# RaptorMai/online-continual-learning

Hardware: NVIDIA H100
Metric: replay-step images/sec (ASER+SCR, ResNet18, CIFAR100) (higher is better)
Workload: dtype f32

## Files before the change

### online-continual-learning_b200/csrc/conv_tc.cu

```cuda
#include <stdlib.h>

#include "conv.cuh"
#include "umma.cuh"

namespace b200ocl {
namespace {

constexpr int TC_THREADS = 128;
constexpr int A_TILE = 128 * 32;

__device__ __forceinline__ void cp_async16(void* smem_dst, const void* gmem_src) {
  const unsigned int s = static_cast<unsigned int>(__cvta_generic_to_shared(smem_dst));
  asm volatile("cp.async.cg.shared.global [%0], [%1], 16;\n" ::"r"(s), "l"(gmem_src));
}

template <int R>
__device__ __forceinline__ void promote(float (&acc)[R], const float (&tmp)[R]) {
#pragma unroll
  for (int i = 0; i < R; ++i) acc[i] += tmp[i];
}

template <int NT>
__device__ __forceinline__ void issue_kblock(float (&d)[2][NT / 2], const float* sAh, const float* sAl, const float* sB) {
  constexpr int B_TILE = NT * 32;
#pragma unroll
  for (int h = 0; h < 2; ++h) {
    const uint64_t dAh = umma::make_smem_desc_sw128(umma::smem_u32(sAh + h * 64 * 32));
    const uint64_t dAl = umma::make_smem_desc_sw128(umma::smem_u32(sAl + h * 64 * 32));
    const uint64_t dBh = umma::make_smem_desc_sw128(umma::smem_u32(sB));
    const uint64_t dBl = umma::make_smem_desc_sw128(umma::smem_u32(sB + B_TILE));
#pragma unroll
    for (int k = 0; k < 4; ++k) {
      const uint64_t adv = (uint64_t)(k * 2);
      umma::mma_tf32_ss<NT>(d[h], dAh + adv, dBh + adv, k > 0 ? 1u : 0u);
      umma::mma_tf32_ss<NT>(d[h], dAh + adv, dBl + adv, 1u);
      umma::mma_tf32_ss<NT>(d[h], dAl + adv, dBh + adv, 1u);
    }
  }
}

template <int NT>
__global__ void __launch_bounds__(TC_THREADS) conv_tc_kernel(ConvArgs a) {
  constexpr int B_TILE = NT * 32;
  constexpr int STAGE_F = 2 * A_TILE + 2 * B_TILE;
  extern __shared__ __align__(1024) unsigned char smem_raw[];
  float* stage0 = reinterpret_cast<float*>(smem_raw);
  __shared__ bool is_last;

  const int tid = threadIdx.x;
  const int bn = a.tc_bn;
  const int n0 = blockIdx.y * bn;
  const int KB = a.tc_kb;
  const int m = blockIdx.x * 128 + tid;
  const bool valid = m < a.M;
  const int hw = a.Hout * a.Wout;
  const int img = valid ? m / hw : 0;
  const int rem = valid ? m - img * hw : 0;
  const int py = rem / a.Wout, px = rem - py * a.Wout;
  const float* wimg = a.w_tc + (size_t)blockIdx.y * KB * 2 * B_TILE;

  float accf[2][NT / 2], tmp[2][NT / 2];
#pragma unroll
  for (int h = 0; h < 2; ++h)
#pragma unroll
    for (int i = 0; i < NT / 2; ++i) accf[h][i] = 0.f;

  int tap = 0, ci = 0;
  const float* tap_src = nullptr;
  auto set_tap = [&]() {
    const int kh = tap / 3, kw = tap - kh * 3;
    const int iy = py + kh - 1, ix = px + kw - 1;
    const bool ok = valid && tap < 9 && (unsigned)iy < (unsigned)a.Hin && (unsigned)ix < (unsigned)a.Win;
    tap_src = ok ? a.in + ((size_t)(img * a.Hin + iy) * a.Win + ix) * a.CK : nullptr;
  };
  set_tap();

  for (int kb = 0; kb < KB; ++kb) {
    const int s = kb & 1;
    float* sAh = stage0 + s * STAGE_F;
    float* sAl = sAh + A_TILE;
    float* sB = sAl + A_TILE;
    const float* bsrc = wimg + (size_t)kb * 2 * B_TILE;
#pragma unroll
    for (int i = 0; i < (2 * B_TILE / 4) / TC_THREADS; ++i)
      cp_async16(sB + (tid + i * TC_THREADS) * 4, bsrc + (tid + i * TC_THREADS) * 4);
// ... 114 lines not shown
      __syncthreads();
      if (is_last) {
        __threadfence();
        const int groups = TC_THREADS / bn;
        const int ch = tid % bn, grp = tid / bn;
        double* s_fin = reinterpret_cast<double*>(stage0);
        __syncthreads();
        if (grp < groups) {
          double s4[4] = {0.0, 0.0, 0.0, 0.0}, q4[4] = {0.0, 0.0, 0.0, 0.0};
          unsigned int b = grp;
          for (; b + 3 * groups < gridDim.x; b += 4 * groups) {
#pragma unroll
            for (int u = 0; u < 4; ++u) {
              const double2 pv = __ldcg(reinterpret_cast<const double2*>(a.stat_part + ((size_t)(b + u * groups) * a.CN + n0 + ch) * 2));
              s4[u] += pv.x;
              q4[u] += pv.y;
            }
          }
          for (; b < gridDim.x; b += groups) {
            const double2 pv = __ldcg(reinterpret_cast<const double2*>(a.stat_part + ((size_t)b * a.CN + n0 + ch) * 2));
            s4[0] += pv.x;
            q4[0] += pv.y;
          }
          s_fin[(grp * bn + ch) * 2 + 0] = (s4[0] + s4[1]) + (s4[2] + s4[3]);
          s_fin[(grp * bn + ch) * 2 + 1] = (q4[0] + q4[1]) + (q4[2] + q4[3]);
        }
        __syncthreads();
        if (tid < bn) {
          double S = 0.0, Q = 0.0;
          for (int g = 0; g < groups; ++g) {
            S += s_fin[(g * bn + tid) * 2 + 0];
            Q += s_fin[(g * bn + tid) * 2 + 1];
          }
          const double cnt = (double)a.M;
          const double mean = S / cnt;
          double var = Q / cnt - mean * mean;
          if (var < 0.0) var = 0.0;
          const int c = n0 + tid;
          a.save_mean[c] = (float)mean;
          a.save_invstd[c] = (float)(1.0 / sqrt(var + (double)a.eps));
          const double unbiased = (a.M > 1) ? var * cnt / (cnt - 1.0) : var;
          a.run_mean[c] = (1.f - a.momentum) * a.run_mean[c] + a.momentum * (float)mean;
          a.run_var[c] = (1.f - a.momentum) * a.run_var[c] + a.momentum * (float)unbiased;
        }
      }
    }
  }
}

template <int NT>
int launch_tc(const ConvArgs& a, cudaStream_t stream) {
  constexpr size_t smem = (size_t)2 * (2 * A_TILE + 2 * NT * 32) * sizeof(float) + 1024;
  static bool configured_dev[B200OCL_MAX_DEVICES] = {};
  bool& configured = configured_dev[b200ocl::device_slot()];
  if (!configured) {
    B200OCL_CUDA(cudaFuncSetAttribute(conv_tc_kernel<NT>, cudaFuncAttributeMaxDynamicSharedMemorySize, (int)smem));
    configured = true;
  }
  dim3 grid((a.M + 127) / 128, a.CN / a.tc_bn);
  B200OCL_PROF(a.flip ? "conv_tc_dgrad" : (a.mode == CONV_EVAL ? "conv_tc_eval" : "conv_tc_train"),
               2.0 * a.M * (double)a.CN * a.CK * 9.0, stream);
  conv_tc_kernel<NT><<<grid, TC_THREADS, smem, stream>>>(a);
  B200OCL_LAUNCHED();
  return B200OCL_OK;
}

}

bool conv_tc_eligible(const ConvArgs& a) {
  static int enabled = -1;
  if (enabled < 0) {
    const char* e = getenv("B200OCL_TC");
    enabled = (e && e[0] == '0') ? 0 : 1;
  }
  if (!enabled || !a.w_tc || a.ks != 3 || a.stride != 1 || a.transposed || a.CK % 20 != 0) return false;
  if (a.Hin != a.Hout || a.Win != a.Wout) return false;
  const long ctas = (long)((a.M + 127) / 128) * (a.CN / a.tc_bn);
  if (ctas < sm_count() / 4) return false;
  if (a.CK == 20 && a.CN == 20 && ctas > 2L * sm_count()) return false;
  return true;
}

int launch_conv_tc(const ConvArgs& a, cudaStream_t stream) {
  const int nt = a.tc_bn <= 20 ? 32 : (a.tc_bn <= 40 ? 48 : 80);
  if (nt == 32) return launch_tc<32>(a, stream);
  if (nt == 48) return launch_tc<48>(a, stream);
  return launch_tc<80>(a, stream);
}

}
```

### online-continual-learning_b200/csrc/conv_tcp.cu

```cuda
#include <stdlib.h>

#include "conv.cuh"
#include "umma.cuh"

namespace b200ocl {
namespace {

constexpr int TP_THREADS = 32 * 13;
constexpr int TP_LOADER_WARP = 9;
constexpr int TP_PS_MAX = 3;
constexpr int TP_BS_MAX = 6;
constexpr int TP_LD_MAX = 13;
constexpr int TP_CONSUMER_WARPS = 8;

using umma::mbar_expect_tx;
using umma::bulk_g2s;

struct TileGeom {
  int wp, pp;
  int tiles_m;
  int prow;
  int pbytes;
};
__host__ __device__ inline TileGeom tile_geom(int N, int H, int W) {
  TileGeom g;
  g.wp = W + 2;
  g.pp = (H + 2) * (W + 2);
  const long last = (long)(N - 1) * g.pp + (long)(H - 1) * g.wp + (W - 1);
  g.tiles_m = (int)(last / 128) + 1;
  g.prow = 128 + 2 * g.wp + 2;
  g.pbytes = (g.prow * 128 + 1023) / 1024 * 1024;
  return g;
}

template <int NT, int KS>
__device__ __forceinline__ void issue_tap(float (&d)[NT / 2], uint64_t dAh, uint64_t dAl, uint64_t dBh, uint64_t dBl) {
  umma::fence();
#pragma unroll
  for (int k = 0; k < KS; ++k) {
    const uint64_t adv = (uint64_t)(k * 2);
    umma::mma_tf32_ss<NT>(d, dAh + adv, dBh + adv, k > 0 ? 1u : 0u);
    umma::mma_tf32_ss<NT>(d, dAh + adv, dBl + adv, 1u);
    umma::mma_tf32_ss<NT>(d, dAl + adv, dBh + adv, 1u);
  }
  umma::commit();
  umma::wait<0>();
  umma::fence_regs(d);
}

template <int NT>
__global__ void __launch_bounds__(TP_THREADS, 1) conv_tcp_kernel(ConvArgs a) {
  constexpr int B_BLOCK = 2 * NT * 32;
  constexpr int R = NT / 2;
  extern __shared__ __align__(1024) unsigned char smem_raw[];
  unsigned char* patch0 = smem_raw;
  __shared__ __align__(8) uint64_t pfull[TP_PS_MAX], pempty[TP_PS_MAX], bfull[9], bempty[TP_BS_MAX];
  __shared__ bool is_last;
  __shared__ int s_fail;
  __shared__ float s_coef[3 * 80];

  const int tid = threadIdx.x, warp = tid >> 5;
  const int bn = a.tp_bn;
  const int n0 = blockIdx.y * bn;
  const int slices = a.tp_slices;
  const TileGeom G = tile_geom(a.N, a.Hin, a.Win);
  const int PS = a.tp_ps, BS = a.tp_bs;
  const int taps_n = a.ks * a.ks;
  const bool one_tap = taps_n == 1;
  float* sB = reinterpret_cast<float*>(smem_raw + (size_t)PS * 2 * G.pbytes);
  const bool resident = (slices == 1 && NT == 32);
  const int b_slots = resident ? 9 : BS;
  float* s_t = sB + (size_t)b_slots * B_BLOCK;
  float* s_acc = s_t + 128 * (bn + 1);

  if (tid == 0) {
    for (int i = 0; i < TP_PS_MAX; ++i) {
      umma::mbar_init(&pfull[i], 128);
      umma::mbar_init(&pempty[i], TP_CONSUMER_WARPS);
    }
    for (int i = 0; i < 9; ++i) umma::mbar_init(&bfull[i], 1);
    for (int i = 0; i < TP_BS_MAX; ++i) umma::mbar_init(&bempty[i], TP_CONSUMER_WARPS);
    umma::fence_mbar_init();
    s_fail = 0;
  }
  __syncthreads();
  const float* wimg = a.w_tp + (size_t)blockIdx.y * slices * taps_n * B_BLOCK;

  if (warp >= TP_LOADER_WARP) {
    const int lt = tid - 32 * TP_LOADER_WARP;
    int pc = 0;
    for (int tile = blockIdx.x; tile < G.tiles_m; tile += gridDim.x) {
      for (int sl = 0; sl < slices; ++sl, ++pc) {
        const int ch_valid = min(32, a.CK - sl * 32);
        const int nch = 2 * ((ch_valid + 7) / 8);
        const int ch = lt & 7, r0 = lt >> 3;
        const int nrow = G.prow;
        const bool ch_live = ch < nch, ch_real = ch * 4 < ch_valid;
        float4 v[TP_LD_MAX];
        int img, yp, xp;
        {
          const int sp = tile * 128 + r0;
          img = sp / G.pp;
          const int rem = sp - img * G.pp;
          yp = rem / G.wp;
          xp = rem - yp * G.wp;
        }
        const int hp = a.Hin + 2;
#pragma unroll
        for (int i = 0; i < TP_LD_MAX; ++i) {
          v[i] = make_float4(0.f, 0.f, 0.f, 0.f);
          const int ri = r0 + 16 * i;
          if (ch_real && ri < nrow) {
            const int y = yp - 1, x = xp - 1;
            if (img < a.N && (unsigned)y < (unsigned)a.Hin && (unsigned)x < (unsigned)a.Win)
              v[i] = __ldg(reinterpret_cast<const float4*>(a.in + ((size_t)(img * a.Hin + y) * a.Win + x) * a.CK + sl * 32) + ch);
          }
          xp += 16;
          while (xp >= G.wp) {
            xp -= G.wp;
            if (++yp == hp) {
              yp = 0;
              ++img;
            }
          }
        }
        const int ps = pc % PS;
        if (!umma::mbar_wait(&pempty[ps], (uint32_t)(((pc / PS) & 1) ^ 1))) s_fail = 1;
        float* ph = reinterpret_cast<float*>(patch0 + (size_t)ps * 2 * G.pbytes);
        float* pl = ph + G.pbytes / 4;
        if (ch_live) {
#pragma unroll
          for (int i = 0; i < TP_LD_MAX; ++i) {
            const int ri = r0 + 16 * i;
            if (ri < nrow) {
              float4 h, l;
              umma::split_tf32(v[i].x, h.x, l.x); umma::split_tf32(v[i].y, h.y, l.y);
              umma::split_tf32(v[i].z, h.z, l.z); umma::split_tf32(v[i].w, h.w, l.w);
              const int off = umma::sw128_offset_f32(ri, ch);
              *reinterpret_cast<float4*>(ph + off) = h;
              *reinterpret_cast<float4*>(pl + off) = l;
            }
          }
        }
        umma::fence_proxy_async_smem();
        umma::mbar_arrive(&pfull[ps]);
      }
    }
  } else if (warp == TP_LOADER_WARP - 1) {
    const uint32_t bytes = (uint32_t)(B_BLOCK * sizeof(float));
    if (resident) {
      if (umma::elect_one_sync()) {
        for (int b = 0; b < taps_n; ++b) {
          mbar_expect_tx(&bfull[b], bytes);
// ... 147 lines not shown
            }
          }
          esync();
          double* s_p = reinterpret_cast<double*>(s_t);
          if (part < parts) {
            s_p[(part * bn + ch) * 2 + 0] = S;
            s_p[(part * bn + ch) * 2 + 1] = Q;
          }
          esync();
          if (et < bn) {
            double Ss = 0.0, Qs = 0.0;
            for (int pp = 0; pp < parts; ++pp) {
              Ss += s_p[(pp * bn + et) * 2 + 0];
              Qs += s_p[(pp * bn + et) * 2 + 1];
            }
            statS += Ss;
            statQ += Qs;
          }
          esync();
        }
      }
    }
    if (epi && a.mode == CONV_TRAIN) {
      if (et < bn) {
        double* dst = a.stat_part + ((size_t)blockIdx.x * a.CN + n0 + et) * 2;
        dst[0] = statS;
        dst[1] = statQ;
      }
      __threadfence();
      esync();
      if (et == 0) is_last = (atomicAdd(a.counter + blockIdx.y, 1u) == gridDim.x - 1);
      esync();
      if (is_last) {
        __threadfence();
        const int groups = 128 / bn;
        const int ch = et % bn, grp = et / bn;
        double* s_fin = reinterpret_cast<double*>(s_t);
        if (grp < groups) {
          double S = 0.0, Q = 0.0;
          unsigned int b = grp;
          for (; b + 3 * groups < gridDim.x; b += 4 * groups) {
            double2 pv[4];
#pragma unroll
            for (int u = 0; u < 4; ++u)
              pv[u] = __ldcg(reinterpret_cast<const double2*>(a.stat_part + ((size_t)(b + u * groups) * a.CN + n0 + ch) * 2));
            S += (pv[0].x + pv[1].x) + (pv[2].x + pv[3].x);
            Q += (pv[0].y + pv[1].y) + (pv[2].y + pv[3].y);
          }
          for (; b < gridDim.x; b += groups) {
            const double2 pv = __ldcg(reinterpret_cast<const double2*>(a.stat_part + ((size_t)b * a.CN + n0 + ch) * 2));
            S += pv.x;
            Q += pv.y;
          }
          s_fin[(grp * bn + ch) * 2 + 0] = S;
          s_fin[(grp * bn + ch) * 2 + 1] = Q;
        }
        esync();
        if (et < bn) {
          double Sm = 0.0, Q = 0.0;
          for (int gq = 0; gq < groups; ++gq) {
            Sm += s_fin[(gq * bn + et) * 2 + 0];
            Q += s_fin[(gq * bn + et) * 2 + 1];
          }
          const double cnt = (double)a.M;
          const double mean = Sm / cnt;
          double var = Q / cnt - mean * mean;
          if (var < 0.0) var = 0.0;
          const int c = n0 + et;
          a.save_mean[c] = (float)mean;
          a.save_invstd[c] = (float)(1.0 / sqrt(var + (double)a.eps));
          const double unbiased = (a.M > 1) ? var * cnt / (cnt - 1.0) : var;
          a.run_mean[c] = (1.f - a.momentum) * a.run_mean[c] + a.momentum * (float)mean;
          a.run_var[c] = (1.f - a.momentum) * a.run_var[c] + a.momentum * (float)unbiased;
        }
      }
    }
  }
  __syncthreads();
  if (s_fail && tid == 0) a.out[(size_t)n0] = __int_as_float(0x7fc00000);
}

template <int NT>
size_t tcp_smem_bytes(const TileGeom& G, int bn, int slices, int ps, int bs) {
  const int b_slots = (slices == 1 && NT == 32) ? 9 : bs;
  return (size_t)ps * 2 * G.pbytes + (size_t)b_slots * 2 * NT * 32 * sizeof(float) +
         (size_t)128 * (bn + 1) * sizeof(float) + (size_t)128 * (NT + 1) * sizeof(float) + 1024;
}

template <int NT>
int launch_tcp(ConvArgs a, cudaStream_t stream) {
  const TileGeom G0 = tile_geom(a.N, a.Hin, a.Win);
  const size_t limit = 227 * 1024 - 4096;
  a.tp_ps = 3; a.tp_bs = 6;
  if (tcp_smem_bytes<NT>(G0, a.tp_bn, a.tp_slices, a.tp_ps, a.tp_bs) > limit) a.tp_bs = 4;
  if (tcp_smem_bytes<NT>(G0, a.tp_bn, a.tp_slices, a.tp_ps, a.tp_bs) > limit) { a.tp_ps = 2; a.tp_bs = 6; }
  const size_t smem = tcp_smem_bytes<NT>(G0, a.tp_bn, a.tp_slices, a.tp_ps, a.tp_bs);
  static size_t configured_dev[B200OCL_MAX_DEVICES] = {};
  size_t& configured = configured_dev[b200ocl::device_slot()];
  if (smem > configured) {
    B200OCL_CUDA(cudaFuncSetAttribute(conv_tcp_kernel<NT>, cudaFuncAttributeMaxDynamicSharedMemorySize, (int)smem));
    configured = smem;
  }
  const TileGeom G = tile_geom(a.N, a.Hin, a.Win);
  const int n_tiles = a.CN / a.tp_bn;
  int gx = sm_count() / n_tiles;
  if (gx < 1) gx = 1;
  if (gx > G.tiles_m) gx = G.tiles_m;
  const int rounds = (G.tiles_m + gx - 1) / gx;
  gx = (G.tiles_m + rounds - 1) / rounds;
  B200OCL_PROF("conv_tcp",
               2.0 * a.M * (double)a.CN * a.CK * 9.0, stream);
  conv_tcp_kernel<NT><<<dim3(gx, n_tiles), TP_THREADS, smem, stream>>>(a);
  B200OCL_LAUNCHED();
  return B200OCL_OK;
}

}

bool conv_tcp_mode_allowed(const ConvArgs& a) {
  static int modes = -1;
  if (modes < 0) {
    const char* m = getenv("B200OCL_TCP_MODES");
    modes = (m && m[0] >= '0' && m[0] <= '7') ? (m[0] - '0') : 5;
  }
  const int bit = a.mode == CONV_EVAL ? 1 : (a.mode == CONV_TRAIN ? 2 : 4);
  return (modes & bit) != 0;
}

bool conv_tcp_eligible(const ConvArgs& a) {
  const char* e = getenv("B200OCL_TCP");
  const char* e2 = getenv("B200OCL_TC");
  const bool enabled = !((e && e[0] == '0') || (e2 && e2[0] == '0'));
  if (!enabled || !a.w_tp || a.transposed || a.CK % 4 != 0) return false;
  if (!((a.ks == 3 && a.pad == 1) || (a.ks == 1 && a.pad == 0))) return false;
  if (a.stride != 1 && (a.stride != 2 || a.flip)) return false;
  if (a.Hout != (a.Hin + 2 * a.pad - a.ks) / a.stride + 1 || a.Wout != (a.Win + 2 * a.pad - a.ks) / a.stride + 1) return false;
  if (128 + 2 * (a.Win + 2) + 2 > 16 * TP_LD_MAX) return false;
  if ((long)a.N * (a.Hin + 2) * (a.Win + 2) > 2000000000L) return false;
  if (a.tp_bn <= 0 || a.tp_bn > 40 || a.CN % a.tp_bn != 0) return false;
  return true;
}

int launch_conv_tcp(const ConvArgs& a, cudaStream_t stream) {
  if (a.tp_bn <= 20) return launch_tcp<32>(a, stream);
  return launch_tcp<48>(a, stream);
}

}
```

### online-continual-learning_b200/csrc/net_plan.cuh

```cuda
#pragma once
#include <stddef.h>
#include <string.h>

#include "../../include/b200ocl.h"

namespace b200ocl {

constexpr int NET_MAX_CONV = 20;
constexpr int NET_MAX_LIN = 3;
constexpr float NET_BN_EPS = 1e-5f;
constexpr float NET_BN_MOMENTUM = 0.1f;

struct ConvL {
  int cin, cout, ks, stride, pad;
  int hin, win, hout, wout;
  size_t w_off;
  size_t pkf_off;
  size_t pkd_off;
  size_t act_off;
  size_t tc_f_off, tc_d_off;
  int tc_kb_f, tc_kb_d;
  int tc_bn_f, tc_bn_d;
  size_t tp_f_off, tp_d_off;
  int tp_sl_f, tp_sl_d;
  int tp_bn_f, tp_bn_d;
};

inline int tc_nt(int bn) { return bn <= 20 ? 32 : (bn <= 40 ? 48 : 80); }
struct BnL {
  int c;
  size_t g_off, b_off;
  size_t stat_off;
  size_t save_off;
};
struct LinL {
  int in, out;
  size_t w_off, b_off;
};
struct BlockL {
  int c1, c2, sc;
};

struct NetPlan {
  int n_conv;
  ConvL conv[NET_MAX_CONV];
  BnL bn[NET_MAX_CONV];
  BlockL blk[8];
  int n_lin;
  LinL lin[NET_MAX_LIN];
  int head;
  int in_h, in_w;
  int final_h, final_w;
  int pooled_h, pooled_w;
  int dim_in;
  int out_dim;
  size_t n_params, n_packed, n_stats, n_bn_channels;
  size_t act_per_image;
  size_t max_act_per_image;
};

inline int conv_out(int x, int ks, int stride, int pad) { return (x + 2 * pad - ks) / stride + 1; }

inline void conv_pack_layout(ConvL& c, size_t& pk, bool tp_all = false) {
  const int cin = c.cin, cout = c.cout, ks = c.ks, stride = c.stride, hin = c.hin, win = c.win;
  c.pkf_off = pk; pk += (size_t)cout * cin * ks * ks;
  c.pkd_off = pk; pk += (size_t)cout * cin * ks * ks;
  c.tc_kb_f = c.tc_kb_d = c.tp_sl_f = c.tp_sl_d = 0;
  if (ks == 3 && stride == 1 && cin % 20 == 0) {
    c.tc_bn_f = cout < 80 ? cout : 80;
    c.tc_bn_d = cin < 80 ? cin : 80;
    c.tc_kb_f = (9 * cin + 31) / 32;
    c.tc_kb_d = (9 * cout + 31) / 32;
    c.tc_f_off = pk; pk += (size_t)(cout / c.tc_bn_f) * c.tc_kb_f * 2 * tc_nt(c.tc_bn_f) * 32;
    c.tc_d_off = pk; pk += (size_t)(cin / c.tc_bn_d) * c.tc_kb_d * 2 * tc_nt(c.tc_bn_d) * 32;
  }
  if (cin % 20 == 0 && win <= 37 && ((ks == 3 && c.pad == 1) || (ks == 1 && c.pad == 0)) &&
      (tp_all || (ks == 3 && stride == 1))) {
    const int taps = ks * ks;
    c.tp_bn_f = cout < 40 ? cout : 40;
    c.tp_sl_f = (cin + 31) / 32;
    c.tp_f_off = pk; pk += (size_t)(cout / c.tp_bn_f) * c.tp_sl_f * taps * 2 * tc_nt(c.tp_bn_f) * 32;
    if (ks == 3 && stride == 1) {
      c.tp_bn_d = cin < 40 ? cin : 40;
      c.tp_sl_d = (cout + 31) / 32;
      c.tp_d_off = pk; pk += (size_t)(cin / c.tp_bn_d) * c.tp_sl_d * 9 * 2 * tc_nt(c.tp_bn_d) * 32;
    }
  }
}

inline int build_plan(const b200ocl_net_desc& d, NetPlan& p) {
  memset(&p, 0, sizeof(p));
  if (d.nf != 20 || d.in_h < 8 || d.in_w < 8 || d.head < 0 || d.head > 3) return B200OCL_EUNSUPPORTED;
  p.head = d.head;
  p.in_h = d.in_h;
  p.in_w = d.in_w;
  size_t off = 0, pk = 0, st = 0, sv = 0, act = 0, max_act = 0;
  int nc = 0;
  auto add_conv = [&](int cin, int cout, int ks, int stride, int hin, int win) {
    ConvL& c = p.conv[nc];
    c.cin = cin; c.cout = cout; c.ks = ks; c.stride = stride; c.pad = (ks == 3) ? 1 : 0;
    c.hin = hin; c.win = win;
    c.hout = conv_out(hin, ks, stride, c.pad);
    c.wout = conv_out(win, ks, stride, c.pad);
    c.w_off = off; off += (size_t)cout * cin * ks * ks;
    conv_pack_layout(c, pk);
    c.act_off = act;
    const size_t a = (size_t)c.hout * c.wout * cout;
    act += a;
    if (a > max_act) max_act = a;
    BnL& b = p.bn[nc];
    b.c = cout;
// ... 60 lines not shown
```

### online-continual-learning_b200/csrc/tc_selftest.cu

```cuda
#include "common.cuh"
#include "umma.cuh"

namespace b200ocl {
namespace {

__global__ void __launch_bounds__(128) wgmma_selftest_kernel(const float* __restrict__ A, const float* __restrict__ B,
                                                             float* __restrict__ D, int N, int K, int mode) {
  extern __shared__ __align__(1024) unsigned char smem_raw[];
  float* sAh = reinterpret_cast<float*>(smem_raw);
  float* sAl = sAh + 64 * 32;
  float* sBh = sAl + 64 * 32;
  float* sBl = sBh + 16 * 32;
  const int tid = threadIdx.x;
  for (int h = 0; h < 2; ++h)
    for (int q = 0; q < N / 16; ++q) {
      float d[8];
#pragma unroll
      for (int i = 0; i < 8; ++i) d[i] = 0.f;
      for (int kb = 0; kb < K / 32; ++kb) {
        for (int idx = tid; idx < (64 + 16) * 8; idx += 128) {
          const int r = idx >> 3, c = idx & 7;
          const bool is_a = r < 64;
          const float* src = is_a ? A + (size_t)(64 * h + r) * K : B + (size_t)(16 * q + r - 64) * K;
          const float4 v = *reinterpret_cast<const float4*>(src + kb * 32 + c * 4);
          float4 hi, lo;
          umma::split_tf32(v.x, hi.x, lo.x); umma::split_tf32(v.y, hi.y, lo.y);
          umma::split_tf32(v.z, hi.z, lo.z); umma::split_tf32(v.w, hi.w, lo.w);
          const int off = umma::sw128_offset_f32(is_a ? r : r - 64, c);
          *reinterpret_cast<float4*>((is_a ? sAh : sBh) + off) = (mode == 0) ? v : hi;
          *reinterpret_cast<float4*>((is_a ? sAl : sBl) + off) = lo;
        }
        umma::fence_proxy_async_smem();
        __syncthreads();
        const uint64_t dAh = umma::make_smem_desc_sw128(umma::smem_u32(sAh));
        const uint64_t dAl = umma::make_smem_desc_sw128(umma::smem_u32(sAl));
        const uint64_t dBh = umma::make_smem_desc_sw128(umma::smem_u32(sBh));
        const uint64_t dBl = umma::make_smem_desc_sw128(umma::smem_u32(sBl));
        umma::fence_regs(d);
        umma::fence();
#pragma unroll
        for (int k = 0; k < 4; ++k) {
          const uint64_t adv = (uint64_t)(k * 2);
          umma::mma_tf32_ss<16>(d, dAh + adv, dBh + adv, (kb > 0 || k > 0) ? 1u : 0u);
          if (mode == 1) {
            umma::mma_tf32_ss<16>(d, dAh + adv, dBl + adv, 1u);
            umma::mma_tf32_ss<16>(d, dAl + adv, dBh + adv, 1u);
          }
        }
        umma::commit();
        umma::wait<0>();
        umma::fence_regs(d);
        __syncthreads();
      }
#pragma unroll
      for (int i = 0; i < 8; ++i)
        D[(size_t)(64 * h + umma::frag_row(tid, i)) * N + 16 * q + umma::frag_col(tid, i)] = d[i];
    }
}

__global__ void __launch_bounds__(128) wgmma_window_kernel(const float* __restrict__ P, const float* __restrict__ B,
                                                           float* __restrict__ D, int rows, int start_row, int sbo_rows,
                                                           int base_off_mode, int N) {
  extern __shared__ __align__(1024) unsigned char smem_raw[];
  float* sP = reinterpret_cast<float*>(smem_raw);
  float* sB = sP + (size_t)((rows + 7) / 8 * 8) * 32;
  const int tid = threadIdx.x;
  for (int idx = tid; idx < rows * 8; idx += 128) {
    const int r = idx >> 3, c = idx & 7;
    *reinterpret_cast<float4*>(sP + umma::sw128_offset_f32(r, c)) = *reinterpret_cast<const float4*>(P + (size_t)r * 32 + c * 4);
  }
  for (int idx = tid; idx < N * 8; idx += 128) {
    const int r = idx >> 3, c = idx & 7;
    *reinterpret_cast<float4*>(sB + umma::sw128_offset_f32(r, c)) = *reinterpret_cast<const float4*>(B + (size_t)r * 32 + c * 4);
  }
  umma::fence_proxy_async_smem();
  __syncthreads();
  for (int h = 0; h < 2; ++h) {
    const int row0 = start_row + 8 * h * sbo_rows;
    uint64_t dA = umma::make_smem_desc_sw128(umma::smem_u32(sP) + (uint32_t)row0 * 128u);
    dA &= ~((uint64_t)0x3FFF << 32);
    dA |= (uint64_t)(((uint32_t)sbo_rows * 128u >> 4) & 0x3FFF) << 32;
    if (base_off_mode == 1) dA |= (uint64_t)(row0 & 7) << 49;
    for (int q = 0; q < N / 16; ++q) {
      const uint64_t dB = umma::make_smem_desc_sw128(umma::smem_u32(sB + q * 16 * 32));
      float d[8];
      umma::fence();
#pragma unroll
      for (int k = 0; k < 4; ++k) {
        const uint64_t adv = (uint64_t)(k * 2);
        umma::mma_tf32_ss<16>(d, dA + adv, dB + adv, k > 0 ? 1u : 0u);
      }
      umma::commit();
      umma::wait<0>();
      umma::fence_regs(d);
#pragma unroll
      for (int i = 0; i < 8; ++i)
        D[(size_t)(64 * h + umma::frag_row(tid, i)) * N + 16 * q + umma::frag_col(tid, i)] = d[i];
    }
  }
}

}
}

extern "C" int b200ocl_selftest_umma_tf32(const float* A, const float* B, float* D, int N, int K, int mode, int* status,
                                          void* stream_) {
  using namespace b200ocl;
  cudaStream_t stream = static_cast<cudaStream_t>(stream_);
  B200OCL_CHECK_ARG(A && B && D && status, "null pointer");
  B200OCL_CHECK_ARG(N >= 16 && N <= 256 && N % 16 == 0 && K >= 32 && K % 32 == 0, "need N in [16,256] %16, K %32");
  const size_t smem = (size_t)(2 * 64 * 32 + 2 * 16 * 32) * sizeof(float) + 1024;
  B200OCL_CUDA(cudaMemsetAsync(status, 0, sizeof(int), stream));
  wgmma_selftest_kernel<<<1, 128, smem, stream>>>(A, B, D, N, K, mode);
  B200OCL_LAUNCHED();
  return B200OCL_OK;
}

extern "C" int b200ocl_selftest_umma_window(const float* P, const float* B, float* D, int rows, int start_row,
                                            int sbo_rows, int base_off_mode, int N, int* status, void* stream_) {
  using namespace b200ocl;
  cudaStream_t stream = static_cast<cudaStream_t>(stream_);
  B200OCL_CHECK_ARG(P && B && D && status, "null pointer");
  B200OCL_CHECK_ARG(N >= 16 && N <= 256 && N % 16 == 0, "need N in [16,256] %16");
  B200OCL_CHECK_ARG(rows > 0 && rows <= 1024 && start_row >= 0 && sbo_rows > 0 &&
                        start_row + 15 * sbo_rows + 8 <= rows,
                    "window exceeds the patch");
  const size_t smem = (size_t)((rows + 7) / 8 * 8 + 256) * 32 * sizeof(float) + 1024;
  B200OCL_CUDA(cudaFuncSetAttribute(wgmma_window_kernel, cudaFuncAttributeMaxDynamicSharedMemorySize, (int)smem));
  B200OCL_CUDA(cudaMemsetAsync(status, 0, sizeof(int), stream));
  wgmma_window_kernel<<<1, 128, smem, stream>>>(P, B, D, rows, start_row, sbo_rows, base_off_mode, N);
  B200OCL_LAUNCHED();
  return B200OCL_OK;
}
```

### online-continual-learning_b200/csrc/umma.cuh

```cuda
#pragma once
#include <stdint.h>

namespace b200ocl {
namespace umma {

__device__ __forceinline__ uint32_t smem_u32(const void* p) {
  return static_cast<uint32_t>(__cvta_generic_to_shared(p));
}

__device__ __forceinline__ int sw128_offset_f32(int row, int chunk16) {
  return (row >> 3) * 256 + (row & 7) * 32 + ((chunk16 ^ (row & 7)) << 2);
}

__device__ __forceinline__ int frag_row(int t, int i) { return ((t >> 5) << 4) + ((t & 31) >> 2) + ((i & 2) << 2); }
__device__ __forceinline__ int frag_col(int t, int i) { return ((i >> 2) << 3) + ((t & 3) << 1) + (i & 1); }

__device__ __forceinline__ uint64_t make_smem_desc_sw128(uint32_t smem_addr) {
  uint64_t d = 0;
  d |= (uint64_t)((smem_addr >> 4) & 0x3FFF);
  d |= (uint64_t)1 << 16;
  d |= (uint64_t)((1024 >> 4) & 0x3FFF) << 32;
  d |= (uint64_t)1 << 62;
  return d;
}

__device__ __forceinline__ void fence() { asm volatile("wgmma.fence.sync.aligned;\n" ::: "memory"); }
__device__ __forceinline__ void commit() { asm volatile("wgmma.commit_group.sync.aligned;\n" ::: "memory"); }
template <int N>
__device__ __forceinline__ void wait() { asm volatile("wgmma.wait_group.sync.aligned %0;\n" ::"n"(N) : "memory"); }
template <int R>
__device__ __forceinline__ void fence_regs(float (&d)[R]) {
#pragma unroll
  for (int i = 0; i < R; ++i) asm volatile("" : "+f"(d[i])::"memory");
}
__device__ __forceinline__ void fence_proxy_async_smem() { asm volatile("fence.proxy.async.shared::cta;\n" ::); }

__device__ __forceinline__ void mbar_init(uint64_t* bar, uint32_t count) {
  asm volatile("mbarrier.init.shared::cta.b64 [%0], %1;\n" ::"r"(smem_u32(bar)), "r"(count));
}
__device__ __forceinline__ void fence_mbar_init() { asm volatile("fence.mbarrier_init.release.cluster;\n" ::); }
__device__ __forceinline__ bool mbar_wait(uint64_t* bar, uint32_t parity, uint32_t max_spins = (1u << 24)) {
  const uint32_t addr = smem_u32(bar);
#pragma unroll 1
  for (uint32_t i = 0; i < max_spins; ++i) {
    uint32_t done;
    asm volatile(
        "{\n\t.reg .pred p;\n\t"
        "mbarrier.try_wait.parity.shared::cta.b64 p, [%1], %2;\n\t"
        "selp.u32 %0, 1, 0, p;\n\t}\n"
        : "=r"(done)
        : "r"(addr), "r"(parity)
        : "memory");
    if (done) return true;
  }
  return false;
}
__device__ __forceinline__ void mbar_arrive(uint64_t* bar) {
  asm volatile("mbarrier.arrive.shared::cta.b64 _, [%0];\n" ::"r"(smem_u32(bar)) : "memory");
}

__device__ __forceinline__ void mbar_expect_tx(uint64_t* bar, uint32_t bytes) {
  asm volatile("mbarrier.arrive.expect_tx.shared::cta.b64 _, [%0], %1;\n" ::"r"(smem_u32(bar)), "r"(bytes)
               : "memory");
}
__device__ __forceinline__ void bulk_g2s(void* smem_dst, const void* gmem_src, uint32_t bytes, uint64_t* bar) {
  asm volatile(
      "cp.async.bulk.shared::cluster.global.mbarrier::complete_tx::bytes [%0], [%1], %2, [%3];\n" ::"r"(
          smem_u32(smem_dst)),
      "l"(gmem_src), "r"(bytes), "r"(smem_u32(bar))
      : "memory");
}

__device__ __forceinline__ bool elect_one_sync() {
  uint32_t pred;
  asm volatile(
      "{\n\t.reg .pred P;\n\t"
      "elect.sync _|P, 0xffffffff;\n\t"
      "selp.u32 %0, 1, 0, P;\n\t}\n"
      : "=r"(pred));
  return pred != 0;
}

template <int N>
__device__ __forceinline__ void mma_tf32_ss(float (&d)[N / 2], uint64_t desc_a, uint64_t desc_b, uint32_t accumulate);
template <int N>
__device__ __forceinline__ void mma_tf32_rs(float (&d)[N / 2], const uint32_t (&a)[4], uint64_t desc_b, uint32_t accumulate);

template <>
__device__ __forceinline__ void mma_tf32_ss<16>(float (&d)[8], uint64_t desc_a, uint64_t desc_b, uint32_t accumulate) {
  asm volatile(
      "{\n\t.reg .pred p;\n\t"
      "setp.ne.b32 p, %10, 0;\n\t"
      "wgmma.mma_async.sync.aligned.m64n16k8.f32.tf32.tf32 {%0,%1,%2,%3,%4,%5,%6,%7}, %8, %9, p, 1, 1;\n\t}\n"
      : "+f"(d[0]), "+f"(d[1]), "+f"(d[2]), "+f"(d[3]), "+f"(d[4]), "+f"(d[5]), "+f"(d[6]), "+f"(d[7])
      : "l"(desc_a), "l"(desc_b), "r"(accumulate));
}

template <>
__device__ __forceinline__ void mma_tf32_ss<32>(float (&d)[16], uint64_t desc_a, uint64_t desc_b, uint32_t accumulate) {
  asm volatile(
      "{\n\t.reg .pred p;\n\t"
      "setp.ne.b32 p, %18, 0;\n\t"
      "wgmma.mma_async.sync.aligned.m64n32k8.f32.tf32.tf32 {%0,%1,%2,%3,%4,%5,%6,%7,%8,%9,%10,%11,%12,%13,%14,%15}, %16, %17, p, 1, 1;\n\t}\n"
      : "+f"(d[0]), "+f"(d[1]), "+f"(d[2]), "+f"(d[3]), "+f"(d[4]), "+f"(d[5]), "+f"(d[6]), "+f"(d[7]), "+f"(d[8]), "+f"(d[9]), "+f"(d[10]), "+f"(d[11]), "+f"(d[12]), "+f"(d[13]), "+f"(d[14]), "+f"(d[15])
      : "l"(desc_a), "l"(desc_b), "r"(accumulate));
}

template <>
__device__ __forceinline__ void mma_tf32_ss<48>(float (&d)[24], uint64_t desc_a, uint64_t desc_b, uint32_t accumulate) {
  asm volatile(
      "{\n\t.reg .pred p;\n\t"
      "setp.ne.b32 p, %26, 0;\n\t"
      "wgmma.mma_async.sync.aligned.m64n48k8.f32.tf32.tf32 {%0,%1,%2,%3,%4,%5,%6,%7,%8,%9,%10,%11,%12,%13,%14,%15,%16,%17,%18,%19,%20,%21,%22,%23}, %24, %25, p, 1, 1;\n\t}\n"
      : "+f"(d[0]), "+f"(d[1]), "+f"(d[2]), "+f"(d[3]), "+f"(d[4]), "+f"(d[5]), "+f"(d[6]), "+f"(d[7]), "+f"(d[8]), "+f"(d[9]), "+f"(d[10]), "+f"(d[11]), "+f"(d[12]), "+f"(d[13]), "+f"(d[14]), "+f"(d[15]), "+f"(d[16]), "+f"(d[17]), "+f"(d[18]), "+f"(d[19]), "+f"(d[20]), "+f"(d[21]), "+f"(d[22]), "+f"(d[23])
      : "l"(desc_a), "l"(desc_b), "r"(accumulate));
}

template <>
__device__ __forceinline__ void mma_tf32_ss<80>(float (&d)[40], uint64_t desc_a, uint64_t desc_b, uint32_t accumulate) {
  asm volatile(
      "{\n\t.reg .pred p;\n\t"
      "setp.ne.b32 p, %42, 0;\n\t"
      "wgmma.mma_async.sync.aligned.m64n80k8.f32.tf32.tf32 {%0,%1,%2,%3,%4,%5,%6,%7,%8,%9,%10,%11,%12,%13,%14,%15,%16,%17,%18,%19,%20,%21,%22,%23,%24,%25,%26,%27,%28,%29,%30,%31,%32,%33,%34,%35,%36,%37,%38,%39}, %40, %41, p, 1, 1;\n\t}\n"
      : "+f"(d[0]), "+f"(d[1]), "+f"(d[2]), "+f"(d[3]), "+f"(d[4]), "+f"(d[5]), "+f"(d[6]), "+f"(d[7]), "+f"(d[8]), "+f"(d[9]), "+f"(d[10]), "+f"(d[11]), "+f"(d[12]), "+f"(d[13]), "+f"(d[14]), "+f"(d[15]), "+f"(d[16]), "+f"(d[17]), "+f"(d[18]), "+f"(d[19]), "+f"(d[20]), "+f"(d[21]), "+f"(d[22]), "+f"(d[23]), "+f"(d[24]), "+f"(d[25]), "+f"(d[26]), "+f"(d[27]), "+f"(d[28]), "+f"(d[29]), "+f"(d[30]), "+f"(d[31]), "+f"(d[32]), "+f"(d[33]), "+f"(d[34]), "+f"(d[35]), "+f"(d[36]), "+f"(d[37]), "+f"(d[38]), "+f"(d[39])
      : "l"(desc_a), "l"(desc_b), "r"(accumulate));
}

template <>
__device__ __forceinline__ void mma_tf32_rs<32>(float (&d)[16], const uint32_t (&a)[4], uint64_t desc_b, uint32_t accumulate) {
  asm volatile(
      "{\n\t.reg .pred p;\n\t"
      "setp.ne.b32 p, %21, 0;\n\t"
      "wgmma.mma_async.sync.aligned.m64n32k8.f32.tf32.tf32 {%0,%1,%2,%3,%4,%5,%6,%7,%8,%9,%10,%11,%12,%13,%14,%15}, {%16,%17,%18,%19}, %20, p, 1, 1;\n\t}\n"
      : "+f"(d[0]), "+f"(d[1]), "+f"(d[2]), "+f"(d[3]), "+f"(d[4]), "+f"(d[5]), "+f"(d[6]), "+f"(d[7]), "+f"(d[8]), "+f"(d[9]), "+f"(d[10]), "+f"(d[11]), "+f"(d[12]), "+f"(d[13]), "+f"(d[14]), "+f"(d[15])
      : "r"(a[0]), "r"(a[1]), "r"(a[2]), "r"(a[3]), "l"(desc_b), "r"(accumulate));
}

__device__ __forceinline__ float round_tf32(float x) {
  uint32_t r;
  asm("cvt.rna.tf32.f32 %0, %1;\n" : "=r"(r) : "f"(x));
  return __uint_as_float(r);
}
__device__ __forceinline__ void split_tf32(float x, float& hi, float& lo) {
  hi = round_tf32(x);
  lo = x - hi;
}

}
}
```

### online-continual-learning_b200/csrc/wgrad_tc.cu

```cuda
#include "common.cuh"
#include "umma.cuh"
#include "wgrad_tc.cuh"

namespace b200ocl {
namespace {

constexpr int WT_THREADS = 32 * 14;
constexpr int WT_PS = 2;
constexpr int WT_LD_MAX = 13;
constexpr int WT_XP = 40;
constexpr int WT_DZ_BYTES = 128 * 128;

struct WtGeom {
  int wp, pp, prow, xbytes;
};
__host__ __device__ inline WtGeom wt_geom(int H, int W) {
  WtGeom g;
  g.wp = W + 2;
  g.pp = (H + 2) * (W + 2);
  g.prow = 128 + 2 * g.wp + 2;
  g.xbytes = ((g.prow + 1) * WT_XP * 4 + 1023) / 1024 * 1024;
  return g;
}

// ... 69 lines not shown
        float* zl = zh + WT_DZ_BYTES / 4;
#pragma unroll
        for (int i = 0; i < 16; ++i) {
          const int pos = r0 + 8 * i;
          const float e[4] = {v[i].x, v[i].y, v[i].z, v[i].w};
#pragma unroll
          for (int j = 0; j < 4; ++j) {
            float h, l;
            umma::split_tf32(e[j], h, l);
            const int off = (pos >> 5) * 1024 + umma::sw128_offset_f32(ch * 4 + j, (pos & 31) >> 2) + (pos & 3);
            zh[off] = h;
            zl[off] = l;
          }
        }
        umma::fence_proxy_async_smem();
        umma::mbar_arrive(&full[ps]);
      }
    }
  } else if (warp >= 8) {
    const int lt = tid - 32 * 8;
    const int ch = lt & 7, r0 = lt >> 3;
    const int ch_valid = min(32, a.Cin - sl * 32);
    const bool ch_real = ch * 4 < ch_valid;
    const int nrow = G.prow;
    const int hp = a.H + 2;
    int pc = 0;
    for (int chain = chain0; chain < chain1; ++chain) {
      const int t1 = min(tiles_m, (chain + 1) * a.tpc);
      for (int tile = chain * a.tpc; tile < t1; ++tile, ++pc) {
        float4 v[WT_LD_MAX];
        int img, yp, xp;
        {
          const int sp = tile * 128 + r0;
          img = sp / G.pp;
          const int rem = sp - img * G.pp;
          yp = rem / G.wp;
          xp = rem - yp * G.wp;
        }
#pragma unroll
        for (int i = 0; i < WT_LD_MAX; ++i) {
          v[i] = make_float4(0.f, 0.f, 0.f, 0.f);
          const int ri = r0 + 16 * i;
          if (ch_real && ri < nrow) {
            const int y = yp - 1, x = xp - 1;
            if (img < a.N && (unsigned)y < (unsigned)a.H && (unsigned)x < (unsigned)a.W)
              v[i] = __ldg(reinterpret_cast<const float4*>(a.x + ((size_t)(img * a.H + y) * a.W + x) * a.Cin + sl * 32) + ch);
          }
          xp += 16;
          while (xp >= G.wp) {
            xp -= G.wp;
            if (++yp == hp) {
              yp = 0;
              ++img;
            }
          }
        }
        const int ps = pc % WT_PS;
        if (!umma::mbar_wait(&empty[ps], (uint32_t)(((pc / WT_PS) & 1) ^ 1))) s_fail = 1;
        float* xs = reinterpret_cast<float*>(smem_raw + (size_t)ps * stage_bytes + 2 * WT_DZ_BYTES);
#pragma unroll
        for (int i = 0; i < WT_LD_MAX; ++i) {
          const int ri = r0 + 16 * i;
          if (ri < nrow) *reinterpret_cast<float4*>(xs + ri * WT_XP + ch * 4) = v[i];
        }
        umma::mbar_arrive(&full[ps]);
      }
    }
  } else {
    const int h = warp >> 2, wt = tid & 127;
    const int m0 = 64 * h + 16 * (warp & 3) + (lane >> 2);
    const int kw = m0 >> 5, c = m0 & 31, q = lane & 3;
    const int n_valid = min(32, a.Cout - cb * 32);
    int pc = 0;
    for (int chain = chain0; chain < chain1; ++chain) {
      float acc[3][16];
      const int t0 = chain * a.tpc, t1 = min(tiles_m, (chain + 1) * a.tpc);
      for (int tile = t0; tile < t1; ++tile, ++pc) {
        const int ps = pc % WT_PS;
        if (!umma::mbar_wait(&full[ps], (uint32_t)((pc / WT_PS) & 1))) s_fail = 1;
        const unsigned char* st = smem_raw + (size_t)ps * stage_bytes;
        const float* xs = reinterpret_cast<const float*>(st + 2 * WT_DZ_BYTES);
        const uint64_t dZ0 = umma::make_smem_desc_sw128(umma::smem_u32(st));
        constexpr uint32_t Z_LO = (uint32_t)WT_DZ_BYTES >> 4;
#pragma unroll 1
        for (int ks = 0; ks < 16; ++ks) {
          const uint64_t dZh = dZ0 + (uint64_t)((ks >> 2) * 256 + (ks & 3) * 2), dZl = dZh + Z_LO;
          uint32_t ah[3][4], al[3][4];
#pragma unroll
          for (int kh = 0; kh < 3; ++kh) load_a(xs, ks * 8 + q + kh * G.wp + kw, c, ah[kh], al[kh]);
          const uint32_t accumulate = (tile == t0 && ks == 0) ? 0u : 1u;
          umma::fence();
#pragma unroll
          for (int kh = 0; kh < 3; ++kh) {
            umma::mma_tf32_rs<32>(acc[kh], ah[kh], dZh, accumulate);
            umma::mma_tf32_rs<32>(acc[kh], ah[kh], dZl, 1u);
            umma::mma_tf32_rs<32>(acc[kh], al[kh], dZh, 1u);
          }
          umma::commit();
          umma::wait<0>();
        }
#pragma unroll
        for (int kh = 0; kh < 3; ++kh) umma::fence_regs(acc[kh]);
        if (lane == 0) umma::mbar_arrive(&empty[ps]);
      }
#pragma unroll
      for (int i = 0; i < 16; i += 2) {
        const int m = 64 * h + umma::frag_row(wt, i), co = umma::frag_col(wt, i);
        const int kwi = m >> 5, ci = sl * 32 + (m & 31);
        if (kwi < 3 && ci < a.Cin && co < n_valid) {
#pragma unroll
          for (int kh = 0; kh < 3; ++kh) {
            float* dst = a.part + ((size_t)chain * k_total + (size_t)(kh * 3 + kwi) * a.Cin + ci) * a.Cout + cb * 32 + co;
            *reinterpret_cast<float2*>(dst) = make_float2(acc[kh][i], acc[kh][i + 1]);
          }
        }
      }
    }
  }
  __syncthreads();
  if (s_fail && tid == 0) a.part[0] = __int_as_float(0x7fc00000);
}

__global__ void wgrad_tc_reduce_kernel(const float* __restrict__ part, int chains, int Cin, int Cout, float* __restrict__ dw) {
  const int e = blockIdx.x * blockDim.x + threadIdx.x;
  const int total = 9 * Cin * Cout;
  if (e >= total) return;
  const int k = e / Cout, co = e - k * Cout;
  const int tap = k / Cin, ci = k - tap * Cin;
  double s = 0.0;
  for (int sp = 0; sp < chains; ++sp) s += (double)part[(size_t)sp * total + e];
  dw[((size_t)co * Cin + ci) * 9 + tap] = (float)s;
}

}

int launch_wgrad_tc(const WgradTcArgs& a, const WgradTcCfg& g, cudaStream_t stream) {
  const WtGeom G = wt_geom(a.H, a.W);
  const size_t smem = (size_t)WT_PS * (2 * WT_DZ_BYTES + (size_t)G.xbytes) + 1024;
  static size_t configured_dev[B200OCL_MAX_DEVICES] = {};
  size_t& configured = configured_dev[device_slot()];
  if (smem > configured) {
    B200OCL_CUDA(cudaFuncSetAttribute(wgrad_tc_kernel, cudaFuncAttributeMaxDynamicSharedMemorySize, (int)smem));
    configured = smem;
  }
  const double M = (double)a.N * a.H * a.W;
  B200OCL_PROF("wgrad_tc", 2.0 * M * 9.0 * a.Cin * a.Cout, stream);
  wgrad_tc_kernel<<<dim3(g.ctas_x, g.slices, g.cout_blocks), WT_THREADS, smem, stream>>>(a, g.tiles);
  B200OCL_LAUNCHED();
  return B200OCL_OK;
}

}

extern "C" size_t b200ocl_wgrad_tc_selftest_workspace_bytes(int N, int H, int W, int cin, int cout) {
  using namespace b200ocl;
  if (N < 1 || H < 1 || W < 1 || cin < 1 || cout < 1) return 0;
  const WgradTcCfg g = wgrad_tc_cfg(N, H, W, 3, 1, 1, cin, cout, sm_count());
  if (!g.eligible) return 0;
  return align_up((size_t)g.chains * 9 * cin * cout * sizeof(float), 256);
}

extern "C" int b200ocl_wgrad_tc_selftest(const float* x, const float* dz, float* dw_oihw, int N, int H, int W, int cin, int cout,
                                         void* workspace, size_t workspace_bytes, void* stream_) {
  using namespace b200ocl;
  cudaStream_t stream = static_cast<cudaStream_t>(stream_);
  B200OCL_CHECK_ARG(x && dz && dw_oihw && N >= 1, "null pointer / empty batch");
  const WgradTcCfg g = wgrad_tc_cfg(N, H, W, 3, 1, 1, cin, cout, sm_count());
  if (!g.eligible) {
    set_error("b200ocl_wgrad_tc_selftest: geometry not covered (3x3 stride 1, W <= 37, channels %% 4 == 0)");
    return B200OCL_EUNSUPPORTED;
  }
  if (!workspace || (reinterpret_cast<uintptr_t>(workspace) & 255) ||
      workspace_bytes < b200ocl_wgrad_tc_selftest_workspace_bytes(N, H, W, cin, cout)) {
    set_error("b200ocl_wgrad_tc_selftest: workspace missing, misaligned or too small");
    return B200OCL_EWORKSPACE;
  }
  WgradTcArgs a{};
  a.x = x; a.dz = dz; a.part = static_cast<float*>(workspace);
  a.N = N; a.H = H; a.W = W; a.Cin = cin; a.Cout = cout;
  a.tpc = g.tpc; a.chains = g.chains; a.chains_per_cta = g.chains_per_cta;
  const int rc = launch_wgrad_tc(a, g, stream);
  if (rc) return rc;
  const int total = 9 * cin * cout;
// ... 5 lines not shown
```

Baseline: 2046.

## Use tighter wgmma N widths and pipeline wgrad MMA groups per tap row

The tensor-core conv kernels now use wgmma N tiles of 24 and 40 instead of 32 and 48 for channel blocks of at most 20 and 40 (counts such as 20, 40 and 80 in this network). This cuts padded MMA work, shared memory and accumulator registers. The wgrad kernel now commits one wgmma group per kh row and waits with wait<2> instead of draining after every k-step, so A-fragment loads overlap in-flight MMAs. The cost is more template variants and a reliance on the async register-fragment ordering being correct.

```diff
diff --git a/online-continual-learning_b200/csrc/conv_tc.cu b/online-continual-learning_b200/csrc/conv_tc.cu
--- a/online-continual-learning_b200/csrc/conv_tc.cu
+++ b/online-continual-learning_b200/csrc/conv_tc.cu
@@ -1,6 +1,7 @@
 #include <stdlib.h>
 
 #include "conv.cuh"
+#include "net_plan.cuh"
 #include "umma.cuh"
 
 namespace b200ocl {
@@ -281,9 +282,9 @@
 }
 
 int launch_conv_tc(const ConvArgs& a, cudaStream_t stream) {
-  const int nt = a.tc_bn <= 20 ? 32 : (a.tc_bn <= 40 ? 48 : 80);
-  if (nt == 32) return launch_tc<32>(a, stream);
-  if (nt == 48) return launch_tc<48>(a, stream);
+  const int nt = tc_nt(a.tc_bn);
+  if (nt == 24) return launch_tc<24>(a, stream);
+  if (nt == 40) return launch_tc<40>(a, stream);
   return launch_tc<80>(a, stream);
 }
 
diff --git a/online-continual-learning_b200/csrc/conv_tcp.cu b/online-continual-learning_b200/csrc/conv_tcp.cu
--- a/online-continual-learning_b200/csrc/conv_tcp.cu
+++ b/online-continual-learning_b200/csrc/conv_tcp.cu
@@ -1,6 +1,7 @@
 #include <stdlib.h>
 
 #include "conv.cuh"
+#include "net_plan.cuh"
 #include "umma.cuh"
 
 namespace b200ocl {
@@ -49,6 +50,9 @@
 }
 
 template <int NT>
+__host__ __device__ constexpr bool tcp_resident(int slices) { return slices == 1 && NT == 24; }
+
+template <int NT>
 __global__ void __launch_bounds__(TP_THREADS, 1) conv_tcp_kernel(ConvArgs a) {
   constexpr int B_BLOCK = 2 * NT * 32;
   constexpr int R = NT / 2;
@@ -68,7 +72,7 @@
   const int taps_n = a.ks * a.ks;
   const bool one_tap = taps_n == 1;
   float* sB = reinterpret_cast<float*>(smem_raw + (size_t)PS * 2 * G.pbytes);
-  const bool resident = (slices == 1 && NT == 32);
+  const bool resident = tcp_resident<NT>(slices);
   const int b_slots = resident ? 9 : BS;
   float* s_t = sB + (size_t)b_slots * B_BLOCK;
   float* s_acc = s_t + 128 * (bn + 1);
@@ -382,7 +386,7 @@
 
 template <int NT>
 size_t tcp_smem_bytes(const TileGeom& G, int bn, int slices, int ps, int bs) {
-  const int b_slots = (slices == 1 && NT == 32) ? 9 : bs;
+  const int b_slots = tcp_resident<NT>(slices) ? 9 : bs;
   return (size_t)ps * 2 * G.pbytes + (size_t)b_slots * 2 * NT * 32 * sizeof(float) +
          (size_t)128 * (bn + 1) * sizeof(float) + (size_t)128 * (NT + 1) * sizeof(float) + 1024;
 }
@@ -442,8 +446,8 @@
 }
 
 int launch_conv_tcp(const ConvArgs& a, cudaStream_t stream) {
-  if (a.tp_bn <= 20) return launch_tcp<32>(a, stream);
-  return launch_tcp<48>(a, stream);
-}
-
-}
+  if (tc_nt(a.tp_bn) == 24) return launch_tcp<24>(a, stream);
+  return launch_tcp<40>(a, stream);
+}
+
+}
diff --git a/online-continual-learning_b200/csrc/net_plan.cuh b/online-continual-learning_b200/csrc/net_plan.cuh
--- a/online-continual-learning_b200/csrc/net_plan.cuh
+++ b/online-continual-learning_b200/csrc/net_plan.cuh
@@ -26,7 +26,7 @@
   int tp_bn_f, tp_bn_d;
 };
 
-inline int tc_nt(int bn) { return bn <= 20 ? 32 : (bn <= 40 ? 48 : 80); }
+inline int tc_nt(int bn) { return bn <= 20 ? 24 : (bn <= 40 ? 40 : 80); }
 struct BnL {
   int c;
   size_t g_off, b_off;
diff --git a/online-continual-learning_b200/csrc/tc_selftest.cu b/online-continual-learning_b200/csrc/tc_selftest.cu
--- a/online-continual-learning_b200/csrc/tc_selftest.cu
+++ b/online-continual-learning_b200/csrc/tc_selftest.cu
@@ -4,24 +4,25 @@
 namespace b200ocl {
 namespace {
 
+template <int NB>
 __global__ void __launch_bounds__(128) wgmma_selftest_kernel(const float* __restrict__ A, const float* __restrict__ B,
                                                              float* __restrict__ D, int N, int K, int mode) {
   extern __shared__ __align__(1024) unsigned char smem_raw[];
   float* sAh = reinterpret_cast<float*>(smem_raw);
   float* sAl = sAh + 64 * 32;
   float* sBh = sAl + 64 * 32;
-  float* sBl = sBh + 16 * 32;
+  float* sBl = sBh + NB * 32;
   const int tid = threadIdx.x;
   for (int h = 0; h < 2; ++h)
-    for (int q = 0; q < N / 16; ++q) {
-      float d[8];
+    for (int q = 0; q < N / NB; ++q) {
+      float d[NB / 2];
 #pragma unroll
-      for (int i = 0; i < 8; ++i) d[i] = 0.f;
+      for (int i = 0; i < NB / 2; ++i) d[i] = 0.f;
       for (int kb = 0; kb < K / 32; ++kb) {
-        for (int idx = tid; idx < (64 + 16) * 8; idx += 128) {
+        for (int idx = tid; idx < (64 + NB) * 8; idx += 128) {
           const int r = idx >> 3, c = idx & 7;
           const bool is_a = r < 64;
-          const float* src = is_a ? A + (size_t)(64 * h + r) * K : B + (size_t)(16 * q + r - 64) * K;
+          const float* src = is_a ? A + (size_t)(64 * h + r) * K : B + (size_t)(NB * q + r - 64) * K;
           const float4 v = *reinterpret_cast<const float4*>(src + kb * 32 + c * 4);
           float4 hi, lo;
           umma::split_tf32(v.x, hi.x, lo.x); umma::split_tf32(v.y, hi.y, lo.y);
@@ -41,10 +42,10 @@
 #pragma unroll
         for (int k = 0; k < 4; ++k) {
           const uint64_t adv = (uint64_t)(k * 2);
-          umma::mma_tf32_ss<16>(d, dAh + adv, dBh + adv, (kb > 0 || k > 0) ? 1u : 0u);
+          umma::mma_tf32_ss<NB>(d, dAh + adv, dBh + adv, (kb > 0 || k > 0) ? 1u : 0u);
           if (mode == 1) {
-            umma::mma_tf32_ss<16>(d, dAh + adv, dBl + adv, 1u);
-            umma::mma_tf32_ss<16>(d, dAl + adv, dBh + adv, 1u);
+            umma::mma_tf32_ss<NB>(d, dAh + adv, dBl + adv, 1u);
+            umma::mma_tf32_ss<NB>(d, dAl + adv, dBh + adv, 1u);
           }
         }
         umma::commit();
@@ -53,8 +54,8 @@
         __syncthreads();
       }
 #pragma unroll
-      for (int i = 0; i < 8; ++i)
-        D[(size_t)(64 * h + umma::frag_row(tid, i)) * N + 16 * q + umma::frag_col(tid, i)] = d[i];
+      for (int i = 0; i < NB / 2; ++i)
+        D[(size_t)(64 * h + umma::frag_row(tid, i)) * N + NB * q + umma::frag_col(tid, i)] = d[i];
     }
 }
 
@@ -108,10 +109,14 @@
   using namespace b200ocl;
   cudaStream_t stream = static_cast<cudaStream_t>(stream_);
   B200OCL_CHECK_ARG(A && B && D && status, "null pointer");
-  B200OCL_CHECK_ARG(N >= 16 && N <= 256 && N % 16 == 0 && K >= 32 && K % 32 == 0, "need N in [16,256] %16, K %32");
-  const size_t smem = (size_t)(2 * 64 * 32 + 2 * 16 * 32) * sizeof(float) + 1024;
+  B200OCL_CHECK_ARG(N >= 16 && N <= 256 && (N % 16 == 0 || N % 24 == 0 || N % 40 == 0) && K >= 32 && K % 32 == 0,
+                    "need N in [16,256] a multiple of 16, 24 or 40, K %32");
+  const int nb = N % 16 == 0 ? 16 : (N % 24 == 0 ? 24 : 40);
+  const size_t smem = (size_t)(2 * 64 * 32 + 2 * nb * 32) * sizeof(float) + 1024;
   B200OCL_CUDA(cudaMemsetAsync(status, 0, sizeof(int), stream));
-  wgmma_selftest_kernel<<<1, 128, smem, stream>>>(A, B, D, N, K, mode);
+  if (nb == 16) wgmma_selftest_kernel<16><<<1, 128, smem, stream>>>(A, B, D, N, K, mode);
+  else if (nb == 24) wgmma_selftest_kernel<24><<<1, 128, smem, stream>>>(A, B, D, N, K, mode);
+  else wgmma_selftest_kernel<40><<<1, 128, smem, stream>>>(A, B, D, N, K, mode);
   B200OCL_LAUNCHED();
   return B200OCL_OK;
 }
diff --git a/online-continual-learning_b200/csrc/umma.cuh b/online-continual-learning_b200/csrc/umma.cuh
--- a/online-continual-learning_b200/csrc/umma.cuh
+++ b/online-continual-learning_b200/csrc/umma.cuh
@@ -97,22 +97,22 @@
 }
 
 template <>
-__device__ __forceinline__ void mma_tf32_ss<32>(float (&d)[16], uint64_t desc_a, uint64_t desc_b, uint32_t accumulate) {
+__device__ __forceinline__ void mma_tf32_ss<24>(float (&d)[12], uint64_t desc_a, uint64_t desc_b, uint32_t accumulate) {
   asm volatile(
       "{\n\t.reg .pred p;\n\t"
-      "setp.ne.b32 p, %18, 0;\n\t"
-      "wgmma.mma_async.sync.aligned.m64n32k8.f32.tf32.tf32 {%0,%1,%2,%3,%4,%5,%6,%7,%8,%9,%10,%11,%12,%13,%14,%15}, %16, %17, p, 1, 1;\n\t}\n"
-      : "+f"(d[0]), "+f"(d[1]), "+f"(d[2]), "+f"(d[3]), "+f"(d[4]), "+f"(d[5]), "+f"(d[6]), "+f"(d[7]), "+f"(d[8]), "+f"(d[9]), "+f"(d[10]), "+f"(d[11]), "+f"(d[12]), "+f"(d[13]), "+f"(d[14]), "+f"(d[15])
+      "setp.ne.b32 p, %14, 0;\n\t"
+      "wgmma.mma_async.sync.aligned.m64n24k8.f32.tf32.tf32 {%0,%1,%2,%3,%4,%5,%6,%7,%8,%9,%10,%11}, %12, %13, p, 1, 1;\n\t}\n"
+      : "+f"(d[0]), "+f"(d[1]), "+f"(d[2]), "+f"(d[3]), "+f"(d[4]), "+f"(d[5]), "+f"(d[6]), "+f"(d[7]), "+f"(d[8]), "+f"(d[9]), "+f"(d[10]), "+f"(d[11])
       : "l"(desc_a), "l"(desc_b), "r"(accumulate));
 }
 
 template <>
-__device__ __forceinline__ void mma_tf32_ss<48>(float (&d)[24], uint64_t desc_a, uint64_t desc_b, uint32_t accumulate) {
+__device__ __forceinline__ void mma_tf32_ss<40>(float (&d)[20], uint64_t desc_a, uint64_t desc_b, uint32_t accumulate) {
   asm volatile(
       "{\n\t.reg .pred p;\n\t"
-      "setp.ne.b32 p, %26, 0;\n\t"
-      "wgmma.mma_async.sync.aligned.m64n48k8.f32.tf32.tf32 {%0,%1,%2,%3,%4,%5,%6,%7,%8,%9,%10,%11,%12,%13,%14,%15,%16,%17,%18,%19,%20,%21,%22,%23}, %24, %25, p, 1, 1;\n\t}\n"
-      : "+f"(d[0]), "+f"(d[1]), "+f"(d[2]), "+f"(d[3]), "+f"(d[4]), "+f"(d[5]), "+f"(d[6]), "+f"(d[7]), "+f"(d[8]), "+f"(d[9]), "+f"(d[10]), "+f"(d[11]), "+f"(d[12]), "+f"(d[13]), "+f"(d[14]), "+f"(d[15]), "+f"(d[16]), "+f"(d[17]), "+f"(d[18]), "+f"(d[19]), "+f"(d[20]), "+f"(d[21]), "+f"(d[22]), "+f"(d[23])
+      "setp.ne.b32 p, %22, 0;\n\t"
+      "wgmma.mma_async.sync.aligned.m64n40k8.f32.tf32.tf32 {%0,%1,%2,%3,%4,%5,%6,%7,%8,%9,%10,%11,%12,%13,%14,%15,%16,%17,%18,%19}, %20, %21, p, 1, 1;\n\t}\n"
+      : "+f"(d[0]), "+f"(d[1]), "+f"(d[2]), "+f"(d[3]), "+f"(d[4]), "+f"(d[5]), "+f"(d[6]), "+f"(d[7]), "+f"(d[8]), "+f"(d[9]), "+f"(d[10]), "+f"(d[11]), "+f"(d[12]), "+f"(d[13]), "+f"(d[14]), "+f"(d[15]), "+f"(d[16]), "+f"(d[17]), "+f"(d[18]), "+f"(d[19])
       : "l"(desc_a), "l"(desc_b), "r"(accumulate));
 }
 
diff --git a/online-continual-learning_b200/csrc/wgrad_tc.cu b/online-continual-learning_b200/csrc/wgrad_tc.cu
--- a/online-continual-learning_b200/csrc/wgrad_tc.cu
+++ b/online-continual-learning_b200/csrc/wgrad_tc.cu
@@ -175,23 +175,23 @@
         const float* xs = reinterpret_cast<const float*>(st + 2 * WT_DZ_BYTES);
         const uint64_t dZ0 = umma::make_smem_desc_sw128(umma::smem_u32(st));
         constexpr uint32_t Z_LO = (uint32_t)WT_DZ_BYTES >> 4;
+        uint32_t ah[3][4], al[3][4];
 #pragma unroll 1
         for (int ks = 0; ks < 16; ++ks) {
           const uint64_t dZh = dZ0 + (uint64_t)((ks >> 2) * 256 + (ks & 3) * 2), dZl = dZh + Z_LO;
-          uint32_t ah[3][4], al[3][4];
-#pragma unroll
-          for (int kh = 0; kh < 3; ++kh) load_a(xs, ks * 8 + q + kh * G.wp + kw, c, ah[kh], al[kh]);
           const uint32_t accumulate = (tile == t0 && ks == 0) ? 0u : 1u;
-          umma::fence();
 #pragma unroll
           for (int kh = 0; kh < 3; ++kh) {
+            umma::wait<2>();
+            load_a(xs, ks * 8 + q + kh * G.wp + kw, c, ah[kh], al[kh]);
+            umma::fence();
             umma::mma_tf32_rs<32>(acc[kh], ah[kh], dZh, accumulate);
             umma::mma_tf32_rs<32>(acc[kh], ah[kh], dZl, 1u);
             umma::mma_tf32_rs<32>(acc[kh], al[kh], dZh, 1u);
-          }
-          umma::commit();
-          umma::wait<0>();
-        }
+            umma::commit();
+          }
+        }
+        umma::wait<0>();
 #pragma unroll
         for (int kh = 0; kh < 3; ++kh) umma::fence_regs(acc[kh]);
         if (lane == 0) umma::mbar_arrive(&empty[ps]);
```

Result: no change. 2064 (median of 6 runs) (+0.9%).
